# saiprasadbarke/robustmvd

Measured on AMD Instinct MI355X. Metric: depth-maps/sec at 768x1152x4srcx256planes; warp+aggregate HBM GB/s vs roofline, higher is better.
Workload: dtype f32; 1 GPU; mvsnet (Path B) forward 768x1152, 4 source views, 256 planes, batch 1 per step (BASELINE.json configs[2]); the regulariser's two layers with 32 input channels (conv0, conv4): every fp32 operand as two range-scaled fp16 terms on fp16 MFMA, fp32 accumulation (at least as close to a float64 convolution as the fp32 matrix instruction over 1e-42..1e30: tests/test_hip_f16.py), the other nine layers and ; parallelism=1 independent replica(s), frames round-robin, no collectives

## Files before the change

### robustmvd_amd/csrc/conv2d_split.hip

```cpp
#include "mvd_common.h"
#include "split_operand.h"
#include <algorithm>
#include <stdlib.h>
#include <string>

#ifndef C2_KO
#define C2_KO 0
#endif

namespace mvd {

constexpr int C2_TH = 16, C2_TW = 16;

template <int KH, int KW, int S, int U8, bool IMG = false>
struct C2Geom {
    static constexpr int CC = 8 * U8;
    static constexpr int PB = 16;
    static constexpr int PH = (C2_TH - 1) * S + KH, PW = (C2_TW - 1) * S + KW;
    static constexpr int PWS = (PW + S - 1) / S;
    static constexpr int ROWB = S * S * PWS * PB;
    static constexpr int C8S = (PH * S * PWS * PB + 255) / 256 * 256;
    static constexpr int PLANE = U8 * C8S;
    static constexpr int UNITS = KH * KW * U8;
    static constexpr int STEPS = (UNITS + 3) / 4;
// ... 190 lines not shown
    }
    return zlive;
}
template <class G, int MTW, class Body>
__device__ __forceinline__ void c2_rows(const char* a, Body&& body) {
    constexpr int PLANE = G::PLANE;
    sph8 xh = *reinterpret_cast<const sph8*>(a), xl = *reinterpret_cast<const sph8*>(a + PLANE);
    sph8 yh = xh, yl = xl;
    if (MTW > 1) {
        yh = *reinterpret_cast<const sph8*>(a + G::ROWB);
        yl = *reinterpret_cast<const sph8*>(a + G::ROWB + PLANE);
    }
#pragma unroll
    for (int m = 0; m < MTW; ++m) {
        const sph8 ch = xh, cl = xl;
        xh = yh; xl = yl;
        if (m + 2 < MTW && !(C2_KO & 8)) {
            yh = *reinterpret_cast<const sph8*>(a + (m + 2) * G::ROWB);
            yl = *reinterpret_cast<const sph8*>(a + (m + 2) * G::ROWB + PLANE);
        }
        body(m, ch, cl);
        __builtin_amdgcn_sched_barrier(0);
    }
}
template <class G, int MTW, int NTW>
__device__ __forceinline__ void c2_kstep(const char* a, const sph8 (&wh)[NTW], const sph8 (&wl)[NTW], spf4 (&acc)[MTW][NTW]) {
    c2_rows<G, MTW>(a, [&](int m, sph8 ch, sph8 cl) __attribute__((always_inline)) {
#pragma unroll
        for (int t = 0; t < NTW; ++t) {
            if (C2_KO & 2) {
                acc[m][t][0] += (float)ch[0] * (float)wh[t][0] + (float)cl[1] * (float)wl[t][1];
                continue;
            }
            acc[m][t] = split_mfma3(wh[t], wl[t], ch, cl, acc[m][t]);
        }
    });
}
template <int MTW, int NT>
__device__ __forceinline__ void c2_finish_rows(const C2Params& p, size_t o0, size_t ostep, int nrows, int cb, const spf4 (&acc)[MTW][NT], int t,
                                               const C2Chan& k, float& amax) {
#pragma unroll
    for (int m = 0; m < MTW; ++m)
        if (m < nrows) c2_finish(p, o0 + m * ostep, cb, acc[m][t], k, amax);
}

template <int KH, int KW, int S, int U8, int WM, int NTW, bool NCHW3>
__global__ void __launch_bounds__(256, 2) conv2d_split_kernel(C2Params p) {
    const float amax_seen = absmax_seen(p.part ? nullptr : p.yamax);
    using G = C2Geom<KH, KW, S, U8, NCHW3>;
    constexpr int WN = 4 / WM, MTW = 16 / WM, STEPS = G::STEPS, PB = G::PB, PLANE = G::PLANE;
    extern __shared__ __attribute__((aligned(16))) char patch[];
    float* const wmax = reinterpret_cast<float*>(patch + 2 * PLANE);
    const int tid = threadIdx.x, lane = tid & 63, wv = tid >> 6;
    const int wm = wv / WN, wn = wv % WN;
    const int g = lane >> 4, px16 = lane & 15;

    const C2Tile tl = c2_tile<S>(p, blockIdx.x);
    const int nb = tl.nb, ks = tl.ks, cls = tl.cls, b = tl.b, od = tl.od, bb = tl.bb;
    const int oy0 = tl.oy0, ox0 = tl.ox0, iy0 = tl.iy0, ix0 = tl.ix0;

    float xsc, xsc_inv;
    split_xscale(p.xamax, xsc, xsc_inv);

    long long goff[G::NIT];
    int loff[G::NIT];
#pragma unroll
    for (int k = 0; k < G::NIT; ++k) {
        const int it = tid + 256 * k;
        const int pix = it / U8, c8 = it % U8;
        const int py = pix / G::PW, pxx = pix % G::PW;
        const int iy = iy0 + py, ix = ix0 + pxx;
        const bool live = it < G::ITEMS;
        const bool inside = live && iy >= 0 && iy < p.Hi && ix >= 0 && ix < p.Wi;
        if constexpr (NCHW3) {
            goff[k] = inside ? ((long long)b * 3 * p.Hi + iy) * p.Wi + ix : -1;
            loff[k] = live ? pix * PB : -1;
        } else {
            goff[k] = inside ? ((long long)iy * p.Wi + ix) * p.xs + c8 * 8 : -1;
            loff[k] = live ? G::lds_byte(py, pxx, c8) : -1;
        }
    }
    int tapoff[STEPS];
    c2_tapoff<G, KW, S, U8, STEPS, NCHW3>(tapoff, g, px16, wm * MTW);

    const int nt0 = nb * (WN * NTW) + wn * NTW;
    const size_t nt_stride = (size_t)p.nchunks * STEPS * 2048;
    const char* wlane = p.wpk + (size_t)cls * p.cls_bytes + (size_t)nt0 * nt_stride + lane * 16;

    spf4 acc[MTW][NTW];
#pragma unroll
    for (int m = 0; m < MTW; ++m)
#pragma unroll
        for (int t = 0; t < NTW; ++t) acc[m][t] = spf4{0, 0, 0, 0};

    const int c_begin = ks * p.chunks_per_split, c_end = min(p.nchunks, c_begin + p.chunks_per_split);

    sph8 wh[NTW], wl[NTW];
    const char* wc = wlane + (size_t)c_begin * STEPS * 2048;
    const char* const wlast = wlane + ((size_t)max(c_end, c_begin + 1) * STEPS - 1) * 2048;
    if (c_begin < c_end) {
#pragma unroll
        for (int t = 0; t < NTW; ++t) split_wpair(wc + t * nt_stride, wh[t], wl[t]);
    }

    for (int chunk = c_begin; chunk < c_end; ++chunk) {
        if (!(C2_KO & 1) || chunk == c_begin) {
            spf4 v0[G::NIT], v1[G::NIT];
            const int kd = chunk / p.nchunks_c, zi = od * p.SD - p.pad_d + kd;
            const bool zlive = zi >= 0 && zi < p.Di;
            const float* xim = p.x + ((size_t)bb * p.Di + (zlive ? zi : 0)) * p.Hi * p.Wi * p.xs + (size_t)(chunk - kd * p.nchunks_c) * G::CC;
#pragma unroll
            for (int k = 0; k < G::NIT; ++k) {
                v0[k] = spf4{0, 0, 0, 0};
                v1[k] = spf4{0, 0, 0, 0};
                if (goff[k] >= 0 && zlive) {
                    if constexpr (NCHW3) {
                        const size_t pl = (size_t)p.Hi * p.Wi;
                        v0[k][0] = p.x[goff[k]]; v0[k][1] = p.x[goff[k] + pl]; v0[k][2] = p.x[goff[k] + 2 * pl];
                    } else {
                        v0[k] = *reinterpret_cast<const spf4*>(xim + goff[k]);
                        v1[k] = *reinterpret_cast<const spf4*>(xim + goff[k] + 4);
                    }
                }
            }
            __syncthreads();
#pragma unroll
            for (int k = 0; k < G::NIT; ++k) {
                if (loff[k] < 0) continue;
                if constexpr (NCHW3) {
                    unsigned h0, h1, l0, l1;
                    split2(xsc, v0[k][0], v0[k][1], h0, l0);
                    split2(xsc, v0[k][2], v0[k][3], h1, l1);
                    *reinterpret_cast<unsigned long long*>(patch + loff[k]) = (unsigned long long)h0 | ((unsigned long long)h1 << 32);
                    *reinterpret_cast<unsigned long long*>(patch + loff[k] + PLANE) = (unsigned long long)l0 | ((unsigned long long)l1 << 32);
                } else {
                    split8_store(patch + loff[k], PLANE, xsc, v0[k], v1[k]);
                }
            }
            __syncthreads();
        }

#pragma unroll
        for (int s = 0; s < STEPS; ++s) {
            sph8 nh[NTW], nl[NTW];
            if (C2_KO & 4) {
#pragma unroll
                for (int t = 0; t < NTW; ++t) { nh[t] = wh[t]; nl[t] = wl[t]; }
            } else {
                const char* wn = wc + 2048;
                wn = wn > wlast ? wlast : wn;
#pragma unroll
                for (int t = 0; t < NTW; ++t) split_wpair(wn + t * nt_stride, nh[t], nl[t]);
                wc += 2048;
            }
            c2_kstep<G, MTW, NTW>(patch + tapoff[s], wh, wl, acc);
#pragma unroll
            for (int t = 0; t < NTW; ++t) { wh[t] = nh[t]; wl[t] = nl[t]; }
        }
    }

    const int ox = ox0 + px16;
    float amax = 0.f;
#pragma unroll
    for (int t = 0; t < NTW; ++t) {
        const int cb = (nt0 + t) * 16 + 4 * g;
        if (p.part) {
            if (ox < p.Wo)
#pragma unroll
                for (int m = 0; m < MTW; ++m) {
                    const int oy = oy0 + wm * MTW + m;
                    if (oy >= p.Ho) continue;
                    const size_t pl = ((size_t)b * p.Ho + oy) * p.Wo + ox;
                    *reinterpret_cast<spf4*>(p.part + (((size_t)cls * p.ksplit + ks) * p.B * p.Ho * p.Wo + pl) * p.ncp + cb) = acc[m][t];
                }
            continue;
        }
        if (cb >= p.Cout || ((C2_KO & 16) && p.B > 1000)) continue;
        const C2Chan kc = c2_chan(p, cb, xsc_inv);
        if (ox < p.Wo) {
            const size_t o0 = c2_out_offset(p, bb, od, oy0 + wm * MTW, ox, cls, cb), ostep = c2_row_step(p);
#pragma unroll
            for (int m = 0; m < MTW; ++m)
                if (oy0 + wm * MTW + m < p.Ho) c2_finish(p, o0 + m * ostep, cb, acc[m][t], kc, amax);
        }
    }
    if (p.yamax && !p.part) {
        for (int o = 32; o > 0; o >>= 1) amax = fmaxf(amax, __shfl_xor(amax, o));
        if (lane == 0) wmax[wv] = amax;
        __syncthreads();
        if (tid == 0) {
            amax = fmaxf(fmaxf(wmax[0], wmax[1]), fmaxf(wmax[2], wmax[3]));
            raise_absmax_seen(p.yamax, amax, amax_seen);
        }
    }
}

template <int KH, int KW, int S, int U8, int WM, int NTW, int WAVES>
__global__ void __launch_bounds__(256, WAVES) conv2d_split_persist_kernel(C2Params p) {
    const float amax_seen = absmax_seen(p.yamax);
    using G = C2Geom<KH, KW, S, U8, false>;
    constexpr int WN = 4 / WM, MTW = 16 / WM, STEPS = G::STEPS, PLANE = G::PLANE;
    extern __shared__ __attribute__((aligned(16))) char patch[];
    float* const wmax = reinterpret_cast<float*>(patch + 2 * PLANE);
    const int tid = threadIdx.x, lane = tid & 63, wv = tid >> 6;
    const int wm = wv / WN, wn = wv % WN;
    const int g = lane >> 4, px16 = lane & 15;
    int t = blockIdx.x;
    if (t >= p.tiles) return;

    float xsc, xsc_inv;
    split_xscale(p.xamax, xsc, xsc_inv);
    int loff[G::NIT];
#pragma unroll
    for (int k = 0; k < G::NIT; ++k) loff[k] = G::item_loff(tid + 256 * k);
    int tapoff[STEPS];
    c2_tapoff<G, KW, S, U8, STEPS, false>(tapoff, g, px16, wm * MTW);
    const size_t nt_stride = (size_t)p.nchunks * STEPS * 2048;
    const size_t plane_floats = (size_t)p.Hi * p.Wi * p.xs;

    int goff[G::NIT];
    spf4 v0[G::NIT], v1[G::NIT];
    bool zlive;
    auto prefetch = [&](const C2Tile& tl, int chunk, bool new_tile) {
        if (new_tile) {
#pragma unroll
            for (int k = 0; k < G::NIT; ++k) goff[k] = (int)G::item_goff(tid + 256 * k, tl.iy0, tl.ix0, p.Hi, p.Wi, p.xs);
        }
        const int kd = chunk / p.nchunks_c, zi = tl.od * p.SD - p.pad_d + kd;
        zlive = c2_prefetch(p.x, (size_t)tl.bb * p.Di, zi, p.Di, plane_floats, (chunk - kd * p.nchunks_c) * G::CC, goff, v0, v1);
    };

    C2Tile tl = c2_tile<S>(p, t);
    prefetch(tl, 0, true);
    C2Chan kc[NTW];
    int nb_have = -1;
    float amax = 0.f;
    for (;;) {
        const int nt0 = tl.nb * (WN * NTW) + wn * NTW;
        const char* const wlane = p.wpk + (size_t)tl.cls * p.cls_bytes + (size_t)nt0 * nt_stride + lane * 16;
        if (tl.nb != nb_have) {
#pragma unroll
            for (int q = 0; q < NTW; ++q) kc[q] = c2_chan(p, (nt0 + q) * 16 + 4 * g, xsc_inv);
            nb_have = tl.nb;
        }
        const int tn = t + (int)gridDim.x;
        const bool more = tn < p.tiles;
        const C2Tile tnext = c2_tile<S>(p, more ? tn : t);

        spf4 acc[MTW][NTW];
#pragma unroll
        for (int m = 0; m < MTW; ++m)
#pragma unroll
            for (int q = 0; q < NTW; ++q) acc[m][q] = spf4{0, 0, 0, 0};

        for (int chunk = 0; chunk < p.nchunks; ++chunk) {
            sph8 wh[STEPS][NTW], wl[STEPS][NTW];
            const char* const wc = wlane + (size_t)chunk * STEPS * 2048;
#pragma unroll
            for (int s = 0; s < STEPS; ++s)
#pragma unroll
                for (int q = 0; q < NTW; ++q) split_wpair(wc + s * 2048 + q * nt_stride, wh[s][q], wl[s][q]);
            __builtin_amdgcn_sched_barrier(0);
            const bool last = chunk + 1 == p.nchunks;
            const bool stage = !(C2_KO & 1) || chunk == 0;
            if (stage) {
                __syncthreads();
#pragma unroll
                for (int k = 0; k < G::NIT; ++k) {
                    if (loff[k] < 0) continue;
                    if (goff[k] < 0 || !zlive) v0[k] = v1[k] = spf4{0, 0, 0, 0};
                    split8_store(patch + loff[k], PLANE, xsc, v0[k], v1[k]);
                }
            }
            __builtin_amdgcn_sched_barrier(0);
            if (!(C2_KO & 1) || last) prefetch(last ? tnext : tl, last ? 0 : chunk + 1, last);
            __builtin_amdgcn_sched_barrier(0);
            if (stage) __syncthreads();
#pragma unroll
            for (int s = 0; s < STEPS; ++s) c2_kstep<G, MTW, NTW>(patch + tapoff[s], wh[s], wl[s], acc);
        }

        const int ox = tl.ox0 + px16;
#pragma unroll
        for (int q = 0; q < NTW; ++q) {
            const int cb = (nt0 + q) * 16 + 4 * g;
            if (cb >= p.Cout || ox >= p.Wo) continue;
            const int oy = tl.oy0 + wm * MTW;
            c2_finish_rows(p, c2_out_offset(p, tl.bb, tl.od, oy, ox, tl.cls, cb), c2_row_step(p), p.Ho - oy, cb, acc, q, kc[q], amax);
        }
        if (!more) break;
        t = tn;
        tl = tnext;
    }
    if (p.yamax) {
        amax = workgroup_max(amax, wmax, tid);
        if (tid == 0) raise_absmax_seen(p.yamax, amax, amax_seen);
    }
}

template <int R>
struct C3Rot {
    static constexpr int value = R;
};
template <int SD, int WAVES, int SLOTS, bool WRES>
__global__ void __launch_bounds__(256, WAVES) conv3d_split_march_kernel(C2Params p) {
    float amax_seen = absmax_seen(p.yamax);
    float* yamax = p.yamax;
    asm volatile("" : "+v"(amax_seen), "+v"(yamax));
    using G = C2Geom<3, 3, SD, 1, false>;
    constexpr int MTW = 4, STEPS = G::STEPS, PLANE = G::PLANE, NSETS = SD == 1 ? 3 : 2;
    extern __shared__ __attribute__((aligned(16))) char patch[];
    float* const wmax = reinterpret_cast<float*>(patch + SLOTS * 2 * PLANE);
    const int tid = threadIdx.x, lane = tid & 63, wv = tid >> 6;
    const int g = lane >> 4, px16 = lane & 15;

    int bx = blockIdx.x;
    const int nb = bx % p.nblocks; bx /= p.nblocks;
    const int tx = bx % p.tiles_x; bx /= p.tiles_x;
    const int ty = bx % p.tiles_y; bx /= p.tiles_y;
    const int od0 = (bx % p.march_runs) * p.march_td, bb = bx / p.march_runs;
    const int nout = min(p.march_td, p.Do - od0);
    const int nplanes = SD == 1 ? nout + 2 : 2 * nout + 1;
    const int z0 = SD * od0 - 1;
    const int oy0 = ty * C2_TH, ox0 = tx * C2_TW, iy0 = oy0 * SD - p.pad_y, ix0 = ox0 * SD - p.pad_x;
    const int ncc = p.nchunks_c;

    float xsc, xsc_inv;
    split_xscale(p.xamax, xsc, xsc_inv);
    int loff[G::NIT], goff[G::NIT];
#pragma unroll
    for (int k = 0; k < G::NIT; ++k) {
        loff[k] = G::item_loff(tid + 256 * k);
        goff[k] = (int)G::item_goff(tid + 256 * k, iy0, ix0, p.Hi, p.Wi, p.xs);
    }
    int tapoff[STEPS];
    c2_tapoff<G, 3, SD, 1, STEPS, false>(tapoff, g, px16, wv * MTW);
    const size_t plane_floats = (size_t)p.Hi * p.Wi * p.xs;
    const char* const wlane = p.wpk + (size_t)nb * p.nchunks * STEPS * 2048 + lane * 16;
    const int cb = nb * 16 + 4 * g, ox = ox0 + px16;
    const C2Chan kc = c2_chan(p, cb, xsc_inv);
    const size_t out0 = c2_out_offset(p, bb, od0, oy0 + wv * MTW, ox, 0, cb), ostep = c2_row_step(p);
    const int nrows = p.Ho - (oy0 + wv * MTW);
    const float* const xrun = p.x + (size_t)bb * p.Di * plane_floats;

    sph8 rh[WRES ? 3 : 1][STEPS], rl[WRES ? 3 : 1][STEPS];
    if constexpr (WRES) {
#pragma unroll
        for (int kd = 0; kd < 3; ++kd)
#pragma unroll
            for (int s = 0; s < STEPS; ++s) split_wpair(wlane + (kd * STEPS + s) * 2048, rh[kd][s], rl[kd][s]);
    }

    spf4 v0[G::NIT], v1[G::NIT];
    int zlive;
    auto prefetch = [&](int z, int c) __attribute__((always_inline)) { zlive = c2_prefetch(xrun, 0, z, p.Di, plane_floats, c * 8, goff, v0, v1); };
    prefetch(z0, 0);

    spf4 acc[MTW][NSETS];
#pragma unroll
    for (int m = 0; m < MTW; ++m)
#pragma unroll
        for (int q = 0; q < NSETS; ++q) acc[m][q] = spf4{0, 0, 0, 0};
    float amax = 0.f;
    int item = 0;

    auto plane = [&](auto rot, int j) __attribute__((always_inline)) {
        constexpr int R = decltype(rot)::value;
        constexpr int SET[3] = {SD == 1 ? R : (R % 2 == 0 ? (R / 2) % 2 : -1), SD == 1 ? (R + 2) % 3 : (R % 2 == 1 ? (R / 2) % 2 : -1),
                                SD == 1 ? (R + 1) % 3 : (R % 2 == 0 ? (R / 2 + 1) % 2 : -1)};
        const int o[3] = {SD == 1 ? j : j / 2, SD == 1 ? j - 1 : (j - 1) / 2, SD == 1 ? j - 2 : j / 2 - 1};
        int on[3], full = 1;
#pragma unroll
        for (int kd = 0; kd < 3; ++kd) {
            on[kd] = (SET[kd] >= 0 && o[kd] >= 0 && o[kd] < nout) ? 1 : 0;
            full &= on[kd] | (SET[kd] < 0 ? 1 : 0);
        }
        for (int c = 0; c < ncc; ++c) {
            sph8 wh[3][STEPS], wl[3][STEPS];
#pragma unroll
            for (int kd = 0; kd < 3; ++kd) {
                if (SET[kd] < 0) continue;
#pragma unroll
                for (int s = 0; s < STEPS; ++s) {
                    if constexpr (WRES) {
                        wh[kd][s] = rh[kd][s]; wl[kd][s] = rl[kd][s];
                    } else {
                        split_wpair(wlane + (size_t)((kd * ncc + c) * STEPS + s) * 2048, wh[kd][s], wl[kd][s]);
                    }
                }
            }
            __builtin_amdgcn_sched_barrier(0);
            char* const slot = patch + (SLOTS == 2 ? (item & 1) * 2 * PLANE : 0);
            if (SLOTS == 1) __syncthreads();
#pragma unroll
            for (int k = 0; k < G::NIT; ++k) {
                if (loff[k] < 0) continue;
                if (goff[k] < 0 || !zlive) v0[k] = v1[k] = spf4{0, 0, 0, 0};
                split8_store(slot + loff[k], PLANE, xsc, v0[k], v1[k]);
            }
            __builtin_amdgcn_sched_barrier(0);
            ++item;
            {
                const bool lastc = c + 1 == ncc, lastp = j + 1 == nplanes;
                prefetch(z0 + j + ((lastc && !lastp) ? 1 : 0), lastc ? (lastp ? c : 0) : c + 1);
            }
            __builtin_amdgcn_sched_barrier(0);
            __syncthreads();
#pragma unroll
            for (int s = 0; s < STEPS; ++s) {
                c2_rows<G, MTW>(slot + tapoff[s], [&](int m, sph8 ch, sph8 cl) __attribute__((always_inline)) {
                    if (full) {
#pragma unroll
                        for (int term = 0; term < 3; ++term)
#pragma unroll
                            for (int kd = 0; kd < 3; ++kd)
                                if (SET[kd] >= 0)
                                    acc[m][max(SET[kd], 0)] = __builtin_amdgcn_mfma_f32_16x16x32_f16(term == 1 ? wl[kd][s] : wh[kd][s], term == 2 ? cl : ch,
                                                                                                     acc[m][max(SET[kd], 0)], 0, 0, 0);
                    } else {
#pragma unroll
                        for (int kd = 0; kd < 3; ++kd)
                            if (on[kd]) {
                                spf4& t = acc[m][max(SET[kd], 0)];
                                t = split_mfma3(wh[kd][s], wl[kd][s], ch, cl, t);
                            }
                    }
                });
            }
        }
        if constexpr (SET[2] >= 0) {
            if (on[2]) {
                if (cb < p.Cout && ox < p.Wo) c2_finish_rows(p, out0 + (size_t)o[2] * p.ys_img, ostep, nrows, cb, acc, SET[2], kc, amax);
#pragma unroll
                for (int m = 0; m < MTW; ++m) acc[m][SET[2]] = spf4{0, 0, 0, 0};
            }
        }
    };
    for (int j = 0; j < nplanes; j += (SD == 1 ? 3 : 4)) {
        plane(C3Rot<0>{}, j);
        if (j + 1 < nplanes) plane(C3Rot<1>{}, j + 1);
        if (j + 2 < nplanes) plane(C3Rot<2>{}, j + 2);
        if constexpr (SD == 2)
            if (j + 3 < nplanes) plane(C3Rot<3>{}, j + 3);
    }
    if (yamax) {
        amax = workgroup_max(amax, wmax, tid);
        if (tid == 0) raise_absmax_seen(yamax, amax, amax_seen);
    }
}

__global__ void __launch_bounds__(256) c2_reduce_kernel(C2Params p) {
    __shared__ float wmax[4];
    const int npix = p.B * p.Ho * p.Wo;
    const int c4n = (p.Cout + 3) / 4;
    const int cls = blockIdx.y;
    float xsc, xsc_inv;
    split_xscale_of(__float_as_uint(*p.xamax), xsc, xsc_inv);
    float amax = 0.f;
    for (int i = blockIdx.x * 256 + threadIdx.x; i < npix * c4n; i += gridDim.x * 256) {
        const int pl = i / c4n;
        const int cb = (i - pl * c4n) * 4;
        const float* pp = p.part + ((size_t)cls * p.ksplit * npix + pl) * p.ncp + cb;
        const size_t kstr = (size_t)npix * p.ncp;
        spf4 s = spf4{0, 0, 0, 0};
        int ks = 0;
        for (; ks + 8 <= p.ksplit; ks += 8) {
            spf4 v[8];
#pragma unroll
            for (int q = 0; q < 8; ++q) v[q] = *reinterpret_cast<const spf4*>(pp + (size_t)(ks + q) * kstr);
#pragma unroll
            for (int q = 0; q < 8; ++q) s += v[q];
        }
        for (; ks + 2 <= p.ksplit; ks += 2) {
            const spf4 v0 = *reinterpret_cast<const spf4*>(pp + (size_t)ks * kstr), v1 = *reinterpret_cast<const spf4*>(pp + (size_t)(ks + 1) * kstr);
            s += v0;
            s += v1;
        }
        const int row = pl / p.Wo, ox = pl - row * p.Wo, b = row / p.Ho, oy = row - b * p.Ho;
        const int bb = p.Do == 1 ? b : b / p.Do, od = b - bb * p.Do;
        c2_finish(p, c2_out_offset(p, bb, od, oy, ox, cls, cb), cb, s, c2_chan(p, cb, xsc_inv), amax);
    }
    if (p.yamax) {
        amax = workgroup_max(amax, wmax, threadIdx.x);
        if (threadIdx.x == 0) raise_absmax(p.yamax, amax);
    }
}

__global__ void __launch_bounds__(256) upsample2x_nhwc_kernel(const float* __restrict__ x, float* __restrict__ y, float* yamax, int B, int C, int h,
                                                              int w, int ys) {
    __shared__ float wmax[4];
    const long long n = (long long)B * 4 * h * w;
    float amax = 0.f;
    for (long long i = (long long)blockIdx.x * 256 + threadIdx.x; i < n; i += (long long)gridDim.x * 256) {
        const int ox = (int)(i % (2 * w)), oy = (int)((i / (2 * w)) % (2 * h)), b = (int)(i / (4LL * h * w));
        const float sy = fmaxf(0.5f * ((float)oy + 0.5f) - 0.5f, 0.f), sx = fmaxf(0.5f * ((float)ox + 0.5f) - 0.5f, 0.f);
        const int y0 = (int)sy, x0 = (int)sx;
        const int y1 = y0 + (y0 < h - 1 ? 1 : 0), x1 = x0 + (x0 < w - 1 ? 1 : 0);
        const float ly1 = sy - (float)y0, ly0 = 1.f - ly1, lx1 = sx - (float)x0, lx0 = 1.f - lx1;
        for (int c = 0; c < C; ++c) {
            const float* pl = x + ((size_t)b * C + c) * h * w;
            const float v = ly0 * (lx0 * pl[(size_t)y0 * w + x0] + lx1 * pl[(size_t)y0 * w + x1]) +
                            ly1 * (lx0 * pl[(size_t)y1 * w + x0] + lx1 * pl[(size_t)y1 * w + x1]);
            y[(size_t)i * ys + c] = v;
            amax = fmaxf(amax, finite_abs_or_zero(v));
        }
    }
    if (yamax) {
        amax = workgroup_max(amax, wmax, threadIdx.x);
        if (threadIdx.x == 0) raise_absmax(yamax, amax);
    }
}

__device__ __forceinline__ int c3_deconv_kidx(int a, int t) { return a == 0 ? (t == 0 ? 1 : -1) : (t == 0 ? 2 : 0); }

__global__ void c3_pack_kernel(const float* __restrict__ w, const float* __restrict__ eun, _Float16* __restrict__ packed, int Cin, int Cout,
                               int U8, int nchunks_c, int ntiles, int steps, int transposed, long long total) {
    const long long e = (long long)blockIdx.x * 256 + threadIdx.x;
    if (e >= total) return;
    const int KD = transposed ? 2 : 3, KP = transposed ? 2 : 3;
    const C2FragIdx f = c2_frag_decode(e, steps, KD * nchunks_c);
    const int j = f.j, term = f.term, unit = 4 * f.step + f.g;
    const int kd = f.chunk / nchunks_c, cc = f.chunk % nchunks_c;
    const int ce = (int)f.rest * 16 + f.row;
    const int tap = unit / U8, cin = cc * 8 * U8 + 8 * (unit % U8) + j;
    const int ncout = transposed ? 8 * Cout : Cout;
    float v = 0.f;
    if (tap < KP * KP && cin < Cin && ce < ncout) {
        const int ty = tap / KP, tx = tap % KP;
        if (transposed) {
            const int k3 = ce / Cout, c = ce % Cout;
            const int kz = c3_deconv_kidx(k3 >> 2, kd), ky = c3_deconv_kidx((k3 >> 1) & 1, ty), kx = c3_deconv_kidx(k3 & 1, tx);
            if (kz >= 0 && ky >= 0 && kx >= 0) v = w[((((size_t)cin * Cout + c) * 3 + kz) * 3 + ky) * 3 + kx];
        } else {
            v = w[((((size_t)ce * Cin + cin) * 3 + kd) * 3 + ty) * 3 + tx];
        }
        v = v / eun[ce];
    }
    _Float16 hi, lo;
    split_weight(v, 1.0f, hi, lo);
    packed[e] = term == 0 ? hi : lo;
}

struct C2Shape {
    int KH, KW, S, U8, steps;
    bool transposed, nchw3;
};

static bool c2_shape(int KH, int KW, int stride, int mode, int cin_pad, C2Shape* s) {
    s->transposed = mode == 1;
    s->nchw3 = mode == 2;
    s->KH = KH; s->KW = KW; s->S = stride;
    if (mode == 1) {
        if (KH != 4 || KW != 4 || stride != 2 || cin_pad % 32) return false;
        s->KH = s->KW = 2; s->S = 1; s->U8 = 4;
    } else if (mode == 2) {
        if (KH != 7 || KW != 7 || stride != 2 || cin_pad != 8) return false;
        s->U8 = 1;
        s->steps = 7;
        return true;
    } else if (KH == 1 && KW == 1 && stride == 1) {
        if (cin_pad % 32) return false;
        s->U8 = 4;
    } else if (KH == 3 && KW == 3 && stride == 1) {
        s->U8 = cin_pad % 32 == 0 ? 4 : 1;
    } else if ((KH == 3 && KW == 3 && stride == 2) || (KH == 5 && KW == 5 && stride == 2)) {
        s->U8 = 1;
    } else {
        return false;
    }
    if (cin_pad % (8 * s->U8)) return false;
    s->steps = (s->KH * s->KW * s->U8 + 3) / 4;
    return true;
}

static int c2_bn(int cout) {
    if (const char* e = exp_env("MVD_C2_BN")) {
        const int v = atoi(e);
        if (v == 16 || v == 32 || v == 64 || v == 128) return v;
    }
    return cout > 64 ? 128 : cout > 32 ? 64 : cout > 16 ? 32 : 16;
}
static int c2_ntiles(int cout) { return (cout + c2_bn(cout) - 1) / c2_bn(cout) * (c2_bn(cout) / 16); }
static size_t c2_frag_bytes(const C2Shape& s, int cin_pad, int cout) {
    const size_t nchunks = (size_t)cin_pad / (8 * s.U8);
    return (s.transposed ? 4 : 1) * (size_t)c2_ntiles(cout) * nchunks * s.steps * 2048;
}
static int c2_cpad(int cout) { return (cout + 127) / 128 * 128; }

struct C2Plan {
    int Ho, Wo, tiles_x, tiles_y, bn, nblocks, ncp, ncls, nchunks, ksplit;
    long long tiles;
    long long persist;
    int march_td;
    size_t part_bytes;
};

enum { C2_K33 = 0, C2_K33W = 1, C2_K33S2 = 2, C2_K55S2 = 3, C2_NOT_PERSISTENT = -1 };
static int c2_persist_kind(const C2Shape& s) {
    if (s.nchw3 || s.transposed) return C2_NOT_PERSISTENT;
    if (s.KH == 3 && s.KW == 3 && s.S == 1) return s.U8 == 4 ? C2_K33W : s.U8 == 1 ? C2_K33 : C2_NOT_PERSISTENT;
    if (s.KH == 3 && s.KW == 3 && s.S == 2 && s.U8 == 1) return C2_K33S2;
    if (s.KH == 5 && s.KW == 5 && s.S == 2 && s.U8 == 1) return C2_K55S2;
    return C2_NOT_PERSISTENT;
}
constexpr int C2_PERSIST_WGS[4][3] = {
    {4, 0, 0},
    {0, 0, 0},
    {0, 0, 0},
    {0, 0, 0},
};
constexpr int C3_MARCH_TD[2][2] = {
    {0, 0},
    {16, 0},
};
constexpr long long C3_MARCH_MIN_WGS = 256;
static int c3_march_forced() {
    const char* e = exp_env("MVD_C3_MARCH");
    return e ? std::max(atoi(e), 0) : 1;
}
static long long c3_march_wgs(const C2Plan& q, int B, int Do, int td) {
    return (long long)q.tiles_x * q.tiles_y * q.nblocks * B * ((Do + td - 1) / td);
}
static int c3_march_td(const C2Shape& s, const C2Plan& q, int B, int Do, int Hi, int Wi, int xs) {
    if (s.KH != 3 || s.U8 != 1 || q.bn != 16 || q.ksplit != 1 || (long long)Hi * Wi * xs > 0x7fffffffLL) return 0;
    if (C2_KO) return 0;
    const int forced = c3_march_forced();
    if (forced != 1) return std::min(forced, Do);
    const int td = std::min(C3_MARCH_TD[s.S - 1][q.nchunks == 3 ? 0 : 1], Do);
    return (td > 0 && c3_march_wgs(q, B, Do, td) >= C3_MARCH_MIN_WGS) ? td : 0;
}
static long long c2_persist_grid(const C2Shape& s, const C2Plan& q, int Hi, int Wi, int xs) {
    const int kind = c2_persist_kind(s);
    if (kind == C2_NOT_PERSISTENT || q.bn > 64 || q.ksplit != 1 || q.tiles > 0x7fffffffLL || (long long)Hi * Wi * xs > 0x7fffffffLL) return 0;
    const int wgs = C2_PERSIST_WGS[kind][q.bn == 16 ? 0 : q.bn == 32 ? 1 : 2];
    if (const char* e = exp_env("MVD_C2_PERSIST")) {
        const long long v = atoll(e);
        if (v <= 0) return 0;
        if (v > 1) return std::min<long long>(v, q.tiles);
    }
    if (wgs == 0) return 0;
    return std::min(q.tiles, (256LL * wgs + q.nblocks - 1) / q.nblocks * q.nblocks);
}
static int c2_ksplit(long long tiles, int nchunks) {
    int ksplit = 1;
    if (tiles < 128)
        while (tiles * ksplit < 320 && ksplit < 32 && nchunks / (ksplit * 2) >= 2) ksplit *= 2;
    if (const char* e = exp_env("MVD_C2_KSPLIT")) {
        const int v = atoi(e);
        if (v >= 1 && v <= 32 && (v & (v - 1)) == 0 && v <= nchunks) ksplit = v;
    }
    return ksplit;
}
static void c2_plan_finish(const C2Shape& s, C2Plan& q, int B, int Hi, int Wi, int xs) {
    q.ksplit = c2_ksplit(q.tiles, q.nchunks);
    q.part_bytes = q.ksplit > 1 ? (size_t)q.ksplit * q.ncls * B * q.Ho * q.Wo * q.ncp * sizeof(float) : 0;
    q.persist = c2_persist_grid(s, q, Hi, Wi, xs);
}
static void c2_plan_tiles(C2Plan& q, int Ho, int Wo, long long images, int cout, int bn) {
    q.Ho = Ho; q.Wo = Wo; q.bn = bn;
    q.tiles_y = (Ho + C2_TH - 1) / C2_TH;
    q.tiles_x = (Wo + C2_TW - 1) / C2_TW;
    q.nblocks = (cout + bn - 1) / bn;
    q.ncp = q.nblocks * bn;
    q.tiles = (long long)q.tiles_x * q.tiles_y * images * q.nblocks;
}
static C2Plan c2_plan(const C2Shape& s, int B, int Hi, int Wi, int cin_pad, int xs, int cout, int KH, int KW, int stride) {
    C2Plan q{};
    q.ncls = s.transposed ? 4 : 1;
    if (s.transposed) c2_plan_tiles(q, Hi, Wi, 4LL * B, cout, c2_bn(cout));
    else c2_plan_tiles(q, (Hi + 2 * (KH / 2) - KH) / stride + 1, (Wi + 2 * (KW / 2) - KW) / stride + 1, B, cout, c2_bn(cout));
    q.nchunks = cin_pad / (8 * s.U8);
    c2_plan_finish(s, q, B, Hi, Wi, xs);
    return q;
}

template <class K>
static int c2_launch_lds(K kern, int lds, long long grid, const C2Params& p, hipStream_t st, const char* what) {
    if (lds > 48 * 1024 && hipFuncSetAttribute((const void*)kern, hipFuncAttributeMaxDynamicSharedMemorySize, lds) != hipSuccess)
        return launch_status((std::string(what) + ": LDS attribute").c_str());
    hipLaunchKernelGGL(kern, dim3((unsigned)grid), dim3(256), lds, st, p);
    return launch_status(what);
}
template <int KH, int KW, int S, int U8, int WM, int NTW, bool NCHW3>
static int c2_launch(const C2Params& p, long long nblk, hipStream_t st) {
    constexpr int lds = 2 * C2Geom<KH, KW, S, U8, NCHW3>::PLANE + 16;
    static_assert(lds <= 80 * 1024, "two workgroups per CU");
    return c2_launch_lds(conv2d_split_kernel<KH, KW, S, U8, WM, NTW, NCHW3>, lds, nblk, p, st, "conv2d_split");
}
template <int KH, int KW, int S, int U8, int WM>
static int c2_launch_persist(const C2Params& p, long long grid, hipStream_t st) {
    using G = C2Geom<KH, KW, S, U8, false>;
    constexpr int WAVES = (G::STEPS == 3 && (G::NIT <= 2 || WM == 4)) ? 3 : 2;
    constexpr int lds = 2 * G::PLANE + 16;
    static_assert(lds <= 48 * 1024, "the persistent form: three workgroups per CU, no LDS attribute");
    return c2_launch_lds(conv2d_split_persist_kernel<KH, KW, S, U8, WM, 1, WAVES>, lds, grid, p, st, "conv2d_split: persistent");
}

template <int SD, int SLOTS, bool WRES>
static int c3_launch_march_as(const C2Params& p, long long grid, hipStream_t st) {
    constexpr int lds = SLOTS * 2 * C2Geom<3, 3, SD, 1, false>::PLANE + 16;
    static_assert(lds <= 80 * 1024, "two workgroups per CU");
    return c2_launch_lds(conv3d_split_march_kernel<SD, 2, SLOTS, WRES>, lds, grid, p, st, "conv3d_split_march");
}
static int c3_launch_march(const C2Shape& s, const C2Params& p, long long grid, hipStream_t st) {
    const bool wres = p.nchunks_c == 1;
#ifdef MVD_EXPERIMENTS
    if (const char* e = exp_env("MVD_C3_SLOTS"); e && atoi(e) == 1) {
        if (s.S == 2) return wres ? c3_launch_march_as<2, 1, true>(p, grid, st) : c3_launch_march_as<2, 1, false>(p, grid, st);
        return wres ? c3_launch_march_as<1, 1, true>(p, grid, st) : c3_launch_march_as<1, 1, false>(p, grid, st);
    }
#endif
    if (s.S == 2 && wres) return c3_launch_march_as<2, 2, true>(p, grid, st);
#ifdef MVD_EXPERIMENTS
    if (s.S == 2) return c3_launch_march_as<2, 2, false>(p, grid, st);
    return wres ? c3_launch_march_as<1, 2, true>(p, grid, st) : c3_launch_march_as<1, 2, false>(p, grid, st);
#else
    return MVD_ERR_INVALID_ARG;
#endif
}

template <int KH, int KW, int S, int U8, bool NCHW3>
static int c2_launch_bn(const C2Params& p, int bn, long long nblk, hipStream_t st) {
    switch (bn) {
        case 128: return c2_launch<KH, KW, S, U8, 1, 2, NCHW3>(p, nblk, st);
        case 64: return c2_launch<KH, KW, S, U8, 1, 1, NCHW3>(p, nblk, st);
        case 32: return c2_launch<KH, KW, S, U8, 2, 1, NCHW3>(p, nblk, st);
        case 16: return c2_launch<KH, KW, S, U8, 4, 1, NCHW3>(p, nblk, st);
    }
    return MVD_ERR_INVALID_ARG;
}
template <int KH, int KW, int S, int U8>
static int c2_launch_persist_bn(const C2Params& p, int bn, long long grid, hipStream_t st) {
    switch (bn) {
#ifdef MVD_EXPERIMENTS
        case 64: return c2_launch_persist<KH, KW, S, U8, 1>(p, grid, st);
        case 32: return c2_launch_persist<KH, KW, S, U8, 2>(p, grid, st);
#endif
        case 16: return c2_launch_persist<KH, KW, S, U8, 4>(p, grid, st);
    }
    return MVD_ERR_INVALID_ARG;
}

static int c2_dispatch(const C2Shape& s, C2Params& p, int bn, long long nblk, long long persist, hipStream_t st) {
    if (persist > 0 && p.ksplit == 1) {
        p.tiles = (int)nblk;
        switch (c2_persist_kind(s)) {
            case C2_K33: return c2_launch_persist_bn<3, 3, 1, 1>(p, bn, persist, st);
#ifdef MVD_EXPERIMENTS
            case C2_K33W: return c2_launch_persist_bn<3, 3, 1, 4>(p, bn, persist, st);
            case C2_K33S2: return c2_launch_persist_bn<3, 3, 2, 1>(p, bn, persist, st);
            case C2_K55S2: return c2_launch_persist_bn<5, 5, 2, 1>(p, bn, persist, st);
#endif
        }
        return MVD_ERR_INVALID_ARG;
    }
    if (s.nchw3) return c2_launch_bn<7, 7, 2, 1, true>(p, bn, nblk, st);
    if (s.KH == 1) return c2_launch_bn<1, 1, 1, 4, false>(p, bn, nblk, st);
    if (s.KH == 2) return s.U8 == 4 ? c2_launch_bn<2, 2, 1, 4, false>(p, bn, nblk, st) : c2_launch_bn<2, 2, 1, 2, false>(p, bn, nblk, st);
    if (s.KH == 5) return c2_launch_bn<5, 5, 2, 1, false>(p, bn, nblk, st);
    if (s.S == 2) return c2_launch_bn<3, 3, 2, 1, false>(p, bn, nblk, st);
    if (s.U8 == 4) return c2_launch_bn<3, 3, 1, 4, false>(p, bn, nblk, st);
    return c2_launch_bn<3, 3, 1, 1, false>(p, bn, nblk, st);
}

static int c2_run(const char* what, const C2Shape& s, C2Params& p, const C2Plan& q, void* workspace, size_t workspace_bytes, hipStream_t st) {
    p.Ho = q.Ho; p.Wo = q.Wo; p.ncls = q.ncls;
    p.tiles_x = q.tiles_x; p.tiles_y = q.tiles_y; p.nblocks = q.nblocks; p.ncp = q.ncp;
    int ksplit = q.ksplit;
    if (ksplit > 1 && (!workspace || workspace_bytes < q.part_bytes)) ksplit = 1;
    p.ksplit = ksplit;
    p.chunks_per_split = (p.nchunks + ksplit - 1) / ksplit;
    p.part = ksplit > 1 ? static_cast<float*>(workspace) : nullptr;
    const long long nblk = q.tiles * ksplit;
    MVD_REQUIRE(nblk <= 0x7fffffffLL, "%s: %lld workgroups exceed the grid limit", what, nblk);
    if (q.march_td > 0) {
        p.march_td = q.march_td;
        p.march_runs = (p.Do + q.march_td - 1) / q.march_td;
        return c3_launch_march(s, p, c3_march_wgs(q, p.B / p.Do, p.Do, q.march_td), st);
    }
    int rc = c2_dispatch(s, p, q.bn, nblk, q.persist, st);
    if (rc != MVD_OK || ksplit == 1) return rc;
    const long long n = (long long)p.B * p.Ho * p.Wo * ((p.Cout + 3) / 4);
    MVD_REQUIRE(n < 0x7fffffffLL, "%s: split reduction over %lld outputs", what, n);
    hipLaunchKernelGGL(c2_reduce_kernel, dim3((unsigned)std::min<long long>((n + 255) / 256, 1024), (unsigned)p.ncls), dim3(256), 0, st, p);
    return launch_status((std::string(what) + ": reduce").c_str());
}

}

extern "C" {

size_t mvd_conv2d_split_packed_weight_bytes(int Cin_pad, int Cout, int KH, int KW, int stride, int mode) {
    mvd::C2Shape s;
    if (Cin_pad <= 0 || Cout <= 0 || !mvd::c2_shape(KH, KW, stride, mode, Cin_pad, &s)) return 0;
    return mvd::c2_frag_bytes(s, Cin_pad, Cout) + (size_t)mvd::c2_cpad(Cout) * sizeof(float);
}

int mvd_pack_conv2d_weights_split(const float* w, int Cin, int Cin_pad, int Cout, int KH, int KW, int stride, int mode, void* packed,
                                  mvd_stream_t stream) {
    MVD_REQUIRE(w && packed, "pack_conv2d_weights_split: NULL argument");
    mvd::C2Shape s;
    MVD_REQUIRE(Cin > 0 && Cin <= Cin_pad && Cout > 0 && mvd::c2_shape(KH, KW, stride, mode, Cin_pad, &s),
                "pack_conv2d_weights_split: layer %dx%d stride %d mode %d with %d (padded %d) -> %d channels is not built", KH, KW, stride, mode,
                Cin, Cin_pad, Cout);
    hipStream_t st = (hipStream_t)stream;
    const size_t fb = mvd::c2_frag_bytes(s, Cin_pad, Cout);
    float* eun = reinterpret_cast<float*>(static_cast<char*>(packed) + fb);
    mvd::split_wscale_launch(w, eun, Cin, Cout, KH * KW, s.transposed, Cout, mvd::c2_cpad(Cout), st);
    const long long total = (long long)(fb / 2);
    hipLaunchKernelGGL(mvd::c2_pack_kernel, dim3((unsigned)((total + 255) / 256)), dim3(256), 0, st, w, eun, (_Float16*)packed, Cin, Cout, s.KH,
                       s.KW, s.U8, Cin_pad / (8 * s.U8), mvd::c2_ntiles(Cout), s.steps, s.transposed ? 1 : s.nchw3 ? 2 : 0, total);
    return mvd::launch_status("pack_conv2d_weights_split");
}

size_t mvd_conv2d_split_workspace_bytes(int B, int Hi, int Wi, int Cin_pad, int Cout, int KH, int KW, int stride, int mode) {
    mvd::C2Shape s;
    if (B <= 0 || Hi <= 0 || Wi <= 0 || Cin_pad <= 0 || Cout <= 0 || !mvd::c2_shape(KH, KW, stride, mode, Cin_pad, &s)) return 0;
    return mvd::c2_plan(s, B, Hi, Wi, Cin_pad, Cin_pad, Cout, KH, KW, stride).part_bytes;
}

int mvd_conv2d_split_f32(const float* x, const float* x_absmax, const void* packed_w, const float* bias, float* y, float* y_absmax, int B,
                         int Hi, int Wi, int Cin_pad, int x_pixel_stride, int Cout, int y_pixel_stride, long long y_row_stride,
                         long long y_image_stride, long long y_channel_stride, int KH, int KW, int stride, int mode, int act, float slope,
                         void* workspace, size_t workspace_bytes, mvd_stream_t stream) {
    MVD_REQUIRE(x && x_absmax && packed_w && y, "conv2d_split: NULL argument");
    MVD_REQUIRE(B > 0 && Hi > 0 && Wi > 0, "conv2d_split: non-positive dimension");
    mvd::C2Shape s;
    MVD_REQUIRE(Cin_pad > 0 && Cout > 0 && mvd::c2_shape(KH, KW, stride, mode, Cin_pad, &s),
                "conv2d_split: layer %dx%d stride %d mode %d with %d -> %d channels is not built", KH, KW, stride, mode, Cin_pad, Cout);
    MVD_REQUIRE(mode == 2 || (x_pixel_stride >= Cin_pad && x_pixel_stride % 4 == 0), "conv2d_split: input pixel stride %d (channels %d)",
                x_pixel_stride, Cin_pad);
    if (y_channel_stride <= 0) y_channel_stride = 1;
    MVD_REQUIRE(y_channel_stride != 1 || y_pixel_stride >= Cout, "conv2d_split: output pixel stride %d below %d channels", y_pixel_stride, Cout);
    MVD_REQUIRE(y_pixel_stride >= 1 && y_row_stride >= 0 && y_image_stride >= 0, "conv2d_split: negative output stride");
    MVD_REQUIRE(act >= 0 && act <= 2, "conv2d_split: act=%d unknown", act);
    MVD_REQUIRE(mode == 2 || (((uintptr_t)x & 15) == 0 && ((uintptr_t)y & 15) == 0), "conv2d_split: x and y must be 16-byte aligned");
    hipStream_t st = (hipStream_t)stream;
    mvd::C2Params p{};
    p.x = x; p.xamax = x_absmax; p.bias = bias; p.y = y; p.yamax = y_absmax;
    p.B = B; p.Hi = Hi; p.Wi = Wi; p.xs = x_pixel_stride; p.nchunks = Cin_pad / (8 * s.U8);
    p.Di = p.Do = p.Dy = p.KD = p.SD = 1; p.pad_d = 0; p.nchunks_c = p.nchunks; p.sub3d = 0; p.Cr = Cout;
    p.Cout = Cout; p.ys = y_pixel_stride; p.act = act; p.slope = slope;
    const size_t fb = mvd::c2_frag_bytes(s, Cin_pad, Cout);
    p.eun = reinterpret_cast<const float*>(static_cast<const char*>(packed_w) + fb);
    const mvd::C2Plan q = mvd::c2_plan(s, B, Hi, Wi, Cin_pad, x_pixel_stride, Cout, KH, KW, stride);
    if (s.transposed) {
        p.Hy = 2 * Hi; p.Wy = 2 * Wi; p.oy_mul = p.ox_mul = 2; p.pad_y = p.pad_x = 1;
    } else {
        p.Hy = q.Ho; p.Wy = q.Wo; p.oy_mul = p.ox_mul = 1; p.pad_y = KH / 2; p.pad_x = KW / 2;
    }
    MVD_REQUIRE(y_channel_stride != 1 || Cout < 4 || (y_pixel_stride % 4 == 0 && y_row_stride % 4 == 0 && y_image_stride % 4 == 0),
                "conv2d_split: channel-last output strides must be multiples of 4 floats");
    p.ycs = y_channel_stride;
    p.ys_row = y_row_stride > 0 ? y_row_stride : (long long)p.Wy * y_pixel_stride;
    p.ys_img = y_image_stride > 0 ? y_image_stride : (long long)p.Hy * p.ys_row;
    p.wpk = static_cast<const char*>(packed_w);
    p.cls_bytes = (long long)(fb / q.ncls);
    return mvd::c2_run("conv2d_split", s, p, q, workspace, workspace_bytes, st);
}

int mvd_upsample2x_nhwc_f32(const float* x, float* y, float* y_absmax, int B, int C, int h, int w, int y_pixel_stride, mvd_stream_t stream) {
    MVD_REQUIRE(x && y, "upsample2x_nhwc: NULL argument");
    MVD_REQUIRE(B > 0 && C > 0 && h > 0 && w > 0 && y_pixel_stride >= C, "upsample2x_nhwc: bad dimension");
    const long long n = (long long)B * 4 * h * w;
    hipLaunchKernelGGL(mvd::upsample2x_nhwc_kernel, dim3((unsigned)std::min<long long>((n + 255) / 256, 1024)), dim3(256), 0, (hipStream_t)stream, x, y,
                       y_absmax, B, C, h, w, y_pixel_stride);
    return mvd::launch_status("upsample2x_nhwc");
}

}

namespace mvd {
static bool c3_shape(int Cin, int Cout, int mode, C2Shape* s, int* ncout) {
    if (Cin <= 0 || Cin % 8 || Cout <= 0 || Cout % 4 || mode < 0 || mode > 2) return false;
    s->transposed = false; s->nchw3 = false;
    if (mode == MVD_DECONV3D_STRIDE2) {
        if (Cin % 16) return false;
        s->KH = s->KW = 2; s->S = 1; s->U8 = Cin % 32 == 0 ? 4 : 2;
        *ncout = 8 * Cout;
    } else {
        s->KH = s->KW = 3; s->S = mode == MVD_CONV3D_STRIDE2 ? 2 : 1;
        s->U8 = (s->S == 1 && Cin % 32 == 0) ? 4 : 1;
        *ncout = Cout;
    }
    s->steps = (s->KH * s->KW * s->U8 + 3) / 4;
    return true;
}
static size_t c3_frag_bytes(const C2Shape& s, int Cin, int ncout, int mode) {
    const size_t KD = mode == MVD_DECONV3D_STRIDE2 ? 2 : 3;
    return (size_t)c2_ntiles(ncout) * KD * (Cin / (8 * s.U8)) * s.steps * 2048;
}
}

extern "C" {

size_t mvd_conv3d_igemm_packed_weight_bytes(int Cin, int Cout, int mode) {
    mvd::C2Shape s;
    int ncout;
    if (!mvd::c3_shape(Cin, Cout, mode, &s, &ncout)) return 0;
    return mvd::c3_frag_bytes(s, Cin, ncout, mode) + (size_t)mvd::c2_cpad(ncout) * sizeof(float);
}

int mvd_pack_conv3d_weights_igemm(const float* w, int Cin, int Cout, int mode, void* packed, mvd_stream_t stream) {
    MVD_REQUIRE(w && packed, "pack_conv3d_weights_igemm: NULL argument");
    mvd::C2Shape s;
    int ncout;
    MVD_REQUIRE(mvd::c3_shape(Cin, Cout, mode, &s, &ncout), "pack_conv3d_weights_igemm: %d -> %d channels, mode %d is not built", Cin, Cout, mode);
    hipStream_t st = (hipStream_t)stream;
    const size_t fb = mvd::c3_frag_bytes(s, Cin, ncout, mode);
    float* eun = reinterpret_cast<float*>(static_cast<char*>(packed) + fb);
    const int tr = mode == MVD_DECONV3D_STRIDE2 ? 1 : 0;
    mvd::split_wscale_launch(w, eun, Cin, Cout, 27, tr != 0, ncout, mvd::c2_cpad(ncout), st);
    const long long total = (long long)(fb / 2);
    hipLaunchKernelGGL(mvd::c3_pack_kernel, dim3((unsigned)((total + 255) / 256)), dim3(256), 0, st, w, eun, (_Float16*)packed, Cin, Cout, s.U8,
                       Cin / (8 * s.U8), mvd::c2_ntiles(ncout), s.steps, tr, total);
    return mvd::launch_status("pack_conv3d_weights_igemm");
}

static mvd::C2Plan c3_plan(const mvd::C2Shape& s, int B, int Di, int Hi, int Wi, int Cin, int ncout, int mode, int* Do) {
    mvd::C2Plan q{};
    const int sd = mode == MVD_CONV3D_STRIDE2 ? 2 : 1;
    *Do = Di / sd; q.ncls = 1;
    int bn = mvd::c2_bn(ncout);
    mvd::c2_plan_tiles(q, Hi / sd, Wi / sd, (long long)B * *Do, ncout, bn);
    const long long planes = q.tiles / q.nblocks;
    if (mode == MVD_CONV3D_STRIDE1 && !mvd::exp_env("MVD_C2_BN") && q.tiles >= 128)
        while (bn > 16 && planes * ((ncout + bn - 1) / bn) < 512) bn /= 2;
    if (mode != MVD_DECONV3D_STRIDE2 && s.U8 == 1 && mvd::c3_march_forced() > 1) bn = 16;
    if (bn != q.bn) mvd::c2_plan_tiles(q, q.Ho, q.Wo, (long long)B * *Do, ncout, bn);
    q.nchunks = (mode == MVD_DECONV3D_STRIDE2 ? 2 : 3) * (Cin / (8 * s.U8));
    mvd::c2_plan_finish(s, q, B * *Do, Hi, Wi, Cin);
    q.march_td = mode == MVD_DECONV3D_STRIDE2 ? 0 : mvd::c3_march_td(s, q, B, *Do, Hi, Wi, Cin);
    return q;
}

size_t mvd_conv3d_igemm_workspace_bytes(int B, int Di, int Hi, int Wi, int Cin, int Cout, int mode) {
    mvd::C2Shape s;
    int ncout, Do;
    if (B <= 0 || Di <= 0 || Hi <= 0 || Wi <= 0 || !mvd::c3_shape(Cin, Cout, mode, &s, &ncout)) return 0;
    return c3_plan(s, B, Di, Hi, Wi, Cin, ncout, mode, &Do).part_bytes;
}

int mvd_conv3d_bn_relu_igemm_f32(const float* x, const float* x_absmax, const void* packed_w, const float* scale, const float* shift,
                                 const float* skip, float* y, float* y_absmax, int B, int Di, int Hi, int Wi, int Cin, int Cout, int mode,
                                 int relu, void* workspace, size_t workspace_bytes, mvd_stream_t stream) {
    MVD_REQUIRE(x && x_absmax && packed_w && scale && shift && y, "conv3d_igemm: NULL argument");
    MVD_REQUIRE(B > 0 && Di > 0 && Hi > 0 && Wi > 0, "conv3d_igemm: non-positive dimension");
    mvd::C2Shape s;
    int ncout;
    MVD_REQUIRE(mvd::c3_shape(Cin, Cout, mode, &s, &ncout), "conv3d_igemm: %d -> %d channels, mode %d is not built", Cin, Cout, mode);
    MVD_REQUIRE(mode != MVD_CONV3D_STRIDE2 || (Di % 2 == 0 && Hi % 2 == 0 && Wi % 2 == 0), "conv3d_igemm stride 2: odd input dims %dx%dx%d", Di, Hi, Wi);
    MVD_REQUIRE((((uintptr_t)x | (uintptr_t)y | (uintptr_t)skip) & 15) == 0, "conv3d_igemm: x, y and skip must be 16-byte aligned");
    hipStream_t st = (hipStream_t)stream;
    int Do;
    const mvd::C2Plan q = c3_plan(s, B, Di, Hi, Wi, Cin, ncout, mode, &Do);
    const bool tr = mode == MVD_DECONV3D_STRIDE2;
    mvd::C2Params p{};
    p.x = x; p.xamax = x_absmax; p.bias = shift; p.scale = scale; p.skip = skip; p.y = y; p.yamax = y_absmax;
    p.wpk = static_cast<const char*>(packed_w);
    p.eun = reinterpret_cast<const float*>(p.wpk + mvd::c3_frag_bytes(s, Cin, ncout, mode));
    p.B = B * Do; p.Hi = Hi; p.Wi = Wi; p.xs = Cin; p.nchunks = q.nchunks;
    p.Di = Di; p.Do = Do; p.KD = tr ? 2 : 3; p.SD = mode == MVD_CONV3D_STRIDE2 ? 2 : 1; p.pad_d = tr ? 0 : 1; p.nchunks_c = Cin / (8 * s.U8);
    p.sub3d = tr ? 1 : 0; p.Cr = Cout; p.Dy = tr ? 2 * Di : Do;
    p.Hy = tr ? 2 * Hi : q.Ho; p.Wy = tr ? 2 * Wi : q.Wo;
    p.oy_mul = p.ox_mul = 1; p.pad_y = p.pad_x = tr ? 0 : 1;
    p.Cout = ncout; p.ys = Cout; p.ycs = 1;
    p.ys_row = (long long)p.Wy * Cout; p.ys_img = (long long)p.Hy * p.ys_row;
    p.cls_bytes = 0;
    p.act = relu ? 2 : 0; p.slope = 0.f;
    MVD_REQUIRE(q.nblocks * (q.bn / 16) <= mvd::c2_ntiles(ncout), "conv3d_igemm: channel tile %d reads past the %d packed fragments", q.bn,
                mvd::c2_ntiles(ncout));
    return mvd::c2_run("conv3d_igemm", s, p, q, workspace, workspace_bytes, st);
}
}
```

Before: 362.7 depth-maps/sec.

## Stage conv3d march weights in LDS and enable marching for stride-1 multi-chunk layers

Adds a WLDS variant of the conv3d depth-marching kernel that copies a workgroup's packed split weights into LDS once, then reads per-step weight fragments from LDS instead of reloading them from global memory on every plane and chunk. It enables the march path for stride-1 layers with more than three channel chunks, within a bounded workgroup count and a depth tile of 10. That path uses one slot at three workgroups per CU. The cost is more LDS per workgroup, single-buffered patches with an extra barrier, and an LDS read plus split inside the step loop.

After: 366.7 depth-maps/sec, median of 5. +1.1%, better.

```diff
diff --git a/robustmvd_amd/csrc/conv2d_split.hip b/robustmvd_amd/csrc/conv2d_split.hip
--- a/robustmvd_amd/csrc/conv2d_split.hip
+++ b/robustmvd_amd/csrc/conv2d_split.hip
@@ -516,8 +516,10 @@
 struct C3Rot {
     static constexpr int value = R;
 };
-template <int SD, int WAVES, int SLOTS, bool WRES>
+constexpr int C3_WLDS_BYTES = 2 * 3 * 3 * 2048;
+template <int SD, int WAVES, int SLOTS, bool WRES, bool WLDS = false>
 __global__ void __launch_bounds__(256, WAVES) conv3d_split_march_kernel(C2Params p) {
+    static_assert(!(WRES && WLDS), "resident weights need no LDS copy");
     float amax_seen = absmax_seen(p.yamax);
     float* yamax = p.yamax;
     asm volatile("" : "+v"(amax_seen), "+v"(yamax));
@@ -525,6 +527,7 @@
     constexpr int MTW = 4, STEPS = G::STEPS, PLANE = G::PLANE, NSETS = SD == 1 ? 3 : 2;
     extern __shared__ __attribute__((aligned(16))) char patch[];
     float* const wmax = reinterpret_cast<float*>(patch + SLOTS * 2 * PLANE);
+    const char* const wfrag = patch + SLOTS * 2 * PLANE + 16 + (threadIdx.x & 63) * 16;
     const int tid = threadIdx.x, lane = tid & 63, wv = tid >> 6;
     const int g = lane >> 4, px16 = lane & 15;
 
@@ -564,6 +567,11 @@
 #pragma unroll
             for (int s = 0; s < STEPS; ++s) split_wpair(wlane + (kd * STEPS + s) * 2048, rh[kd][s], rl[kd][s]);
     }
+    if constexpr (WLDS) {
+        const char* const wsrc = p.wpk + (size_t)nb * p.nchunks * STEPS * 2048;
+        char* const wdst = patch + SLOTS * 2 * PLANE + 16;
+        for (int i = tid * 16; i < p.nchunks * STEPS * 2048; i += 256 * 16) *reinterpret_cast<spf4*>(wdst + i) = *reinterpret_cast<const spf4*>(wsrc + i);
+    }
 
     spf4 v0[G::NIT], v1[G::NIT];
     int zlive;
@@ -598,8 +606,8 @@
                 for (int s = 0; s < STEPS; ++s) {
                     if constexpr (WRES) {
                         wh[kd][s] = rh[kd][s]; wl[kd][s] = rl[kd][s];
-                    } else {
-                        split_wpair(wlane + (size_t)((kd * ncc + c) * STEPS + s) * 2048, wh[kd][s], wl[kd][s]);
+                    } else if constexpr (!WLDS) {
+                        split_wpair(wlane + (size_t)(((C2_KO & 32) ? 0 : (kd * ncc + c) * STEPS) + s) * 2048, wh[kd][s], wl[kd][s]);
                     }
                 }
             }
@@ -622,6 +630,11 @@
             __syncthreads();
 #pragma unroll
             for (int s = 0; s < STEPS; ++s) {
+                if constexpr (WLDS) {
+#pragma unroll
+                    for (int kd = 0; kd < 3; ++kd)
+                        if (SET[kd] >= 0) split_wpair(wfrag + ((kd * ncc + c) * STEPS + s) * 2048, wh[kd][s], wl[kd][s]);
+                }
                 c2_rows<G, MTW>(slot + tapoff[s], [&](int m, sph8 ch, sph8 cl) __attribute__((always_inline)) {
                     if (full) {
 #pragma unroll
@@ -824,10 +837,12 @@
     {0, 0, 0},
 };
 constexpr int C3_MARCH_TD[2][2] = {
-    {0, 0},
+    {0, 10},
     {16, 0},
 };
 constexpr long long C3_MARCH_MIN_WGS = 256;
+constexpr long long C3_MARCH_LDS_MAX_WGS = 768;
+static bool c3_wlds_fits(int nchunks) { return nchunks > 3 && nchunks * 3 * 2048 <= C3_WLDS_BYTES; }
 static int c3_march_forced() {
     const char* e = exp_env("MVD_C3_MARCH");
     return e ? std::max(atoi(e), 0) : 1;
@@ -837,11 +852,14 @@
 }
 static int c3_march_td(const C2Shape& s, const C2Plan& q, int B, int Do, int Hi, int Wi, int xs) {
     if (s.KH != 3 || s.U8 != 1 || q.bn != 16 || q.ksplit != 1 || (long long)Hi * Wi * xs > 0x7fffffffLL) return 0;
-    if (C2_KO) return 0;
+    if (C2_KO & ~32) return 0;
     const int forced = c3_march_forced();
     if (forced != 1) return std::min(forced, Do);
+    if (q.nchunks != 3 && !c3_wlds_fits(q.nchunks)) return 0;
     const int td = std::min(C3_MARCH_TD[s.S - 1][q.nchunks == 3 ? 0 : 1], Do);
-    return (td > 0 && c3_march_wgs(q, B, Do, td) >= C3_MARCH_MIN_WGS) ? td : 0;
+    const long long wgs = td > 0 ? c3_march_wgs(q, B, Do, td) : 0;
+    if (q.nchunks != 3 && wgs > C3_MARCH_LDS_MAX_WGS) return 0;
+    return wgs >= C3_MARCH_MIN_WGS ? td : 0;
 }
 static long long c2_persist_grid(const C2Shape& s, const C2Plan& q, int Hi, int Wi, int xs) {
     const int kind = c2_persist_kind(s);
@@ -910,16 +928,25 @@
     return c2_launch_lds(conv2d_split_persist_kernel<KH, KW, S, U8, WM, 1, WAVES>, lds, grid, p, st, "conv2d_split: persistent");
 }
 
-template <int SD, int SLOTS, bool WRES>
+template <int SD, int SLOTS, bool WRES, bool WLDS = false, int WAVES = 2>
 static int c3_launch_march_as(const C2Params& p, long long grid, hipStream_t st) {
-    constexpr int lds = SLOTS * 2 * C2Geom<3, 3, SD, 1, false>::PLANE + 16;
-    static_assert(lds <= 80 * 1024, "two workgroups per CU");
-    return c2_launch_lds(conv3d_split_march_kernel<SD, 2, SLOTS, WRES>, lds, grid, p, st, "conv3d_split_march");
+    constexpr int lds = SLOTS * 2 * C2Geom<3, 3, SD, 1, false>::PLANE + 16 + (WLDS ? C3_WLDS_BYTES : 0);
+    static_assert(lds * WAVES <= 160 * 1024, "WAVES workgroups per CU");
+    return c2_launch_lds(conv3d_split_march_kernel<SD, WAVES, SLOTS, WRES, WLDS>, lds, grid, p, st, "conv3d_split_march");
 }
 static int c3_launch_march(const C2Shape& s, const C2Params& p, long long grid, hipStream_t st) {
     const bool wres = p.nchunks_c == 1;
+    bool wlds = c3_wlds_fits(p.nchunks);
 #ifdef MVD_EXPERIMENTS
-    if (const char* e = exp_env("MVD_C3_SLOTS"); e && atoi(e) == 1) {
+    int slots = 0;
+    if (const char* e = exp_env("MVD_C3_WLDS")) wlds = wlds && atoi(e) != 0;
+    if (const char* e = exp_env("MVD_C3_SLOTS")) slots = atoi(e);
+    if (wlds && s.S == 2) return c3_launch_march_as<2, 1, false, true>(p, grid, st);
+    if (wlds && slots == 2) return c3_launch_march_as<1, 2, false, true>(p, grid, st);
+#endif
+    if (wlds && s.S == 1) return c3_launch_march_as<1, 1, false, true, 3>(p, grid, st);
+#ifdef MVD_EXPERIMENTS
+    if (slots == 1) {
         if (s.S == 2) return wres ? c3_launch_march_as<2, 1, true>(p, grid, st) : c3_launch_march_as<2, 1, false>(p, grid, st);
         return wres ? c3_launch_march_as<1, 1, true>(p, grid, st) : c3_launch_march_as<1, 1, false>(p, grid, st);
     }
```
